# soberguo/HOIGen

Measured on AMD Instinct MI355X. Metric: union-crop embeddings/sec ViT-B/16 bs=256, higher is better.
Workload: dtype f16; 1 GPU; CLIP ViT-B/16 union-region encode (encode_image), 224x224 crops, batch 256 per GPU, synthetic N(0,1) crops + seeded synthetic weights (BASELINE.json configs[1]); last_block=all rows (option last_block_row0 = 0), batch_per_gpu=256, global_batch=256, parallelism=dp1

## Files before the change

hoigen_amd/csrc/hg_api.hip:

```cpp
#include <limits.h>

#include "hg_host.h"
#include "hg_preproc_geom.h"

namespace {

struct Option { const char *key, *env; int hg_ctx::*member; bool is_switch; int lo = 0, hi = 1; const char* want = nullptr; bool say_got = true; };
const Option OPTIONS[] = {
    {"chunk_rows", "HG_CHUNK_ROWS", &hg_ctx::max_chunk_rows, false, 256, INT_MAX, ">= 256", false},
    {"last_block_row0", "HG_LAST_BLOCK_ROW0", &hg_ctx::opt_row0, true},
    {"ln_fuse", "HG_LN_FUSE", &hg_ctx::opt_ln_fuse, true},
    {"adapter_fuse", "HG_ADAPTER_FUSE", &hg_ctx::opt_adapter_fuse, true},
    {"adapter_fold", "HG_ADAPTER_FOLD", &hg_ctx::opt_adapter_fold, true},
    {"stream_hilo", "HG_STREAM_HILO", &hg_ctx::opt_stream_hilo, true},
    {"adapter_long", "HG_ADAPTER_LONG", &hg_ctx::opt_adapter_long, true},
    {"qkv_attn", "HG_QKV_ATTN", &hg_ctx::opt_qkv_attn, false, 0, 2, "0, 1 or 2"},
    {"qkv_attn_text", "HG_QKV_ATTN_TEXT", &hg_ctx::opt_qkv_attn_text, false, 0, 2, "0, 1 or 2"},
    {"qkv_attn_min_seq", "HG_QKV_ATTN_MIN_SEQ", &hg_ctx::opt_qkv_attn_min_seq, false, 1, INT_MAX, ">= 1"},
    {"qkv_attn_gsz", "HG_QKV_ATTN_GSZ", &hg_ctx::opt_qkv_attn_gsz, false, 0, 6, "0 .. 6"},
    {"qkv_attn_c", "HG_QKV_ATTN_C", &hg_ctx::opt_qkv_attn_c, false, 0, 1, "0 or 1"},
    {"text_ln_fold", "HG_TEXT_LN_FOLD", &hg_ctx::opt_text_ln_fold, false, 0, 2, "0, 1 or 2"},
    {"vae_fused", "HG_VAE_FUSED", &hg_ctx::opt_vae_fused, false, 0, 2, "0, 1 or 2"},
    {"mlp_pair", "HG_MLP_PAIR", &hg_ctx::opt_mlp_pair, false, 0, 1, "0 or 1"},
    {"mlp_pair_chunk", "HG_MLP_PAIR_CHUNK", &hg_ctx::opt_mlp_pair_chunk, false, 1, 64, "1 .. 64"},
    {"mlp_pair_fc_slots", "HG_MLP_PAIR_FC_SLOTS", &hg_ctx::opt_mlp_pair_fc_slots, false, 1, 64, "1 .. 64"},
    {"mlp_pair256", "HG_MLP_PAIR256", &hg_ctx::opt_mlp_pair256, false, 0, 1, "0 or 1"},
    {"mlp_pair256_min_m", "HG_MLP_PAIR256_MIN_M", &hg_ctx::opt_mlp_pair256_min_m, false, 2048, INT_MAX, ">= 2048"},
    {"mlp_pair256_chunk", "HG_MLP_PAIR256_CHUNK", &hg_ctx::opt_mlp_pair256_chunk, false, 1, 64, "1 .. 64"},
    {"mlp_pair256_ratio", "HG_MLP_PAIR256_RATIO", &hg_ctx::opt_mlp_pair256_ratio, false, 1, 8, "1 .. 8"},
    {"mlp_pair256_launches", "HG_MLP_PAIR256_LAUNCHES", &hg_ctx::n_pair256_launches, false, 0, INT_MAX, ">= 0"},
    {"mlp_pair_fault", "HG_MLP_PAIR_FAULT", &hg_ctx::opt_mlp_pair_fault, false, 0, 1, "0 or 1"},
};
const Option* find_option(const char* key) {
    for (const Option& o : OPTIONS)
        if (!strcmp(o.key, key)) return &o;
    return nullptr;
}

}

extern "C" {

const char* hg_version(void) { return "hoigen_amd 0.1 (gfx950)"; }

// ... 245 lines not shown
```

hoigen_amd/csrc/hg_gemm_ring_body.h:

```cpp
#pragma once
#include <type_traits>

#include "hg_gemm_dev.h"

namespace hg {

#ifdef HG_STAMPS
#ifndef HG_STAMP_MASK
#define HG_STAMP_MASK 0xFF
#endif
#define SEG_B(k) do { if constexpr ((HG_STAMP_MASK >> (k)) & 1) t_beg = __builtin_amdgcn_s_memtime(); } while (0)
#define SEG_E(k) do { if constexpr ((HG_STAMP_MASK >> (k)) & 1) tacc[k] += __builtin_amdgcn_s_memtime() - t_beg; } while (0)
#else
#define SEG_B(k) do {} while (0)
#define SEG_E(k) do {} while (0)
#endif

template <int MF, int EPI, bool PH2, int HL = 0, class SCHED>
__device__ __forceinline__ void gemm_ring_body(const GemmArgs& p, const unsigned a_bytes, const int mode, const SCHED& sc) {
#if defined(__HIP_DEVICE_COMPILE__)
    constexpr int BM = 64 * MF, BK = 64;
    constexpr int AH = MF * 4096, BH = 16384;
    constexpr int STAGE = 2 * AH + 2 * BH;
    constexpr int GA = MF / 2, GB = 2;
    static_assert(GA <= 2, "DMA piece helpers cover two pieces per half-tile");
    constexpr int N1 = 2 * GA + 3 * GB, N2 = 3 * GA + 2 * GB;
    constexpr bool RLN = (EPI == EPI_RESID_LN_F32);
    constexpr bool RESID = (EPI == EPI_BIAS_RESID_F32 || EPI == EPI_SCALE_RESID_F32 || RLN);
    constexpr bool F16_STORES = (EPI == EPI_BIAS_F16 || EPI == EPI_BIAS_QGELU_F16 || EPI == EPI_BIAS_RELU_F16 ||
                                 EPI == EPI_LN_BIAS_F16 || EPI == EPI_LN_BIAS_QGELU_F16);
    constexpr bool IN_HL = (HL == 2 || HL == 3), OUT_HL = (HL == 2);
    static_assert(HL == 0 || (IN_HL && RLN && MF == 4 && !PH2), "hi / lo stream: EPI_RESID_LN_F32 on 256 rows, four phases, hl 2 or 3");
    constexpr int E_RAW = IN_HL ? (OUT_HL ? 40 : 88) : RLN ? 8 * MF + 4 * MF + 2 * MF : (F16_STORES ? 4 * MF : 8 * MF);
    constexpr int E = E_RAW > 52 ? 52 : E_RAW;
    constexpr bool XPRE = RESID && MF == 2;
    constexpr bool LNC = (EPI == EPI_LN_BIAS_F16 || EPI == EPI_LN_BIAS_QGELU_F16);
    constexpr bool ROLL = RESID && MF == 4;
    constexpr int ROLL_W = RLN ? 6 : 8;
    constexpr int R = XPRE ? E : (IN_HL ? 12 : ROLL ? ROLL_W + (RLN ? 1 : 0) : 0);
    constexpr bool PUB = SCHED::PUBLISH;
    static_assert(!PUB || (PH2 && (EPI == EPI_LN_BIAS_F16 || EPI == EPI_LN_BIAS_QGELU_F16)), "hand-off: two-phase loop, fp16 LayerNorm-fold epilogues");
    constexpr int BIAS_OFF = 2 * STAGE;
    const int MR_OFF = BIAS_OFF + 2 * p.N * 4;
    extern __shared__ __attribute__((aligned(16))) char smem[];
#ifdef HG_STAMPS
    unsigned long long tacc[8] = {0, 0, 0, 0, 0, 0, 0, 0}, t_beg = 0, t_all = 0;
#endif
    const int tid = sc.thread_id(), lane = tid & 63;
    const int wave = __builtin_amdgcn_readfirstlane(tid >> 6);
    const int wm = wave >> 2, wn = wave & 3;
    const int nk = p.K / BK;

    const int bid = blockIdx.x;
    const int n_items = sc.n_items();
    const int my_tiles = n_items;
    const int tiles_m_all = (p.M + BM - 1) / BM;
    auto item_get = [&](int e, int& tm, int& tn, int& kb, int& ke) {
        kb = 0;
        ke = nk;
        sc.tile(e, tm, tn);
    };
    {
        const int dunit = mode >> 8;
// ... 78 lines not shown
    half8 xa[MF][2], wb[2][2][2];
    auto read_A = [&](int h, int buf) {
#pragma unroll
        for (int f = 0; f < MF; ++f)
#pragma unroll
            for (int ks = 0; ks < 2; ++ks)
                xa[f][ks] = *reinterpret_cast<const half8*>(smem + buf + h * AH + a_row + f * 2048 + coff[ks]);
    };
    auto read_W = [&](auto H, int buf) {
        constexpr int h = decltype(H)::value;
#pragma unroll
        for (int g2 = 0; g2 < 2; ++g2)
#pragma unroll
            for (int ks = 0; ks < 2; ++ks)
                wb[h][g2][ks] = *reinterpret_cast<const half8*>(smem + buf + h * BH + w_row + g2 * 2048 + coff[ks]);
    };

    f32x4 acc[2][2][MF][2];
    auto zero_acc = [&]() {
#pragma unroll
        for (int a = 0; a < 2; ++a)
#pragma unroll
            for (int b = 0; b < 2; ++b)
#pragma unroll
                for (int f = 0; f < MF; ++f)
#pragma unroll
                    for (int g2 = 0; g2 < 2; ++g2) acc[a][b][f][g2] = f32x4{0.f, 0.f, 0.f, 0.f};
    };
    auto mma = [&](auto HA, auto HB) {
        constexpr int ha = decltype(HA)::value, hb = decltype(HB)::value;
// ... 111 lines not shown
            }
        };
        auto chunk_row = [&](int rg) {
            int m = m0 + (rg / MF) * (BM / 2) + wm * MF * 16 + (rg % MF) * 16 + (lane & 15);
            return m < p.M ? m : p.M - 1;
        };
        auto chunk_load = [&](int c) {
            const int rg = c >> 2, hb = (c >> 1) & 1, g2 = c & 1;
            const int n = n0 + hb * 128 + wn * 32 + g2 * 16 + 4 * (lane >> 4);
            return *reinterpret_cast<const f32x4*>(reinterpret_cast<const float*>(p.out) + (size_t)chunk_row(rg) * p.ldc + n);
        };
        auto ph2_ktile = [&](auto KIND_T) {
            constexpr int KINDX = decltype(KIND_T)::value;
            constexpr int KIND = KINDX >= 4 ? 0 : KINDX;
            const int buf = (g & 1) * STAGE;
            const bool post = post_ok;
            const bool more = KIND < 2 || r + 1 < n_items;
            const bool pub = PUB && r > 0 && wave == 0;
            (void)post; (void)more; (void)pub;
            constexpr int NP = 2 * GA + 2 * GB;
            read_A(0, buf);
            read_W(I0{}, buf);
            read_W(I1{}, buf);
            if constexpr (LNC && KIND == 2) {
                if (lane < BM / 16)
                    __builtin_amdgcn_raw_ptr_buffer_load_lds(rsM, (HG_LDS void*)(smem + MR_OFF + wave * BM), 16, lane * 16,
                                                             (m0 + wave * (BM / 8)) * 8, 0, 0);
            }
            if (KIND < 3 || more) issue_A(1, 0, GA);
            if constexpr (ROLL && KIND == 3) {
                {
#pragma unroll
                    for (int c = 0; c < ROLL_W; ++c) xw[c] = chunk_load(c);
                    if constexpr (RLN) muw[0] = p.mu[chunk_row(0)];
                }
            }
            if constexpr (XPRE && KIND == 3) {
                {
#pragma unroll
                    for (int ha = 0; ha < 2; ++ha)
#pragma unroll
                        for (int f = 0; f < MF; ++f) {
                            int m = m0 + ha * (BM / 2) + wm * MF * 16 + f * 16 + (lane & 15);
                            m = m < p.M ? m : p.M - 1;
#pragma unroll
                            for (int hb = 0; hb < 2; ++hb)
#pragma unroll
                                for (int g2 = 0; g2 < 2; ++g2) {
                                    const int n = n0 + hb * 128 + wn * 32 + g2 * 16 + 4 * (lane >> 4);
                                    xres[ha][hb][f][g2] = *reinterpret_cast<const f32x4*>(
                                        reinterpret_cast<const float*>(p.out) + (size_t)m * p.ldc + n);
                                }
                        }
                }
            }
            SEG_B(0);
            if constexpr (KINDX == 5) { if (pub) wait_vm<NP + 1>(); else wait_vm<NP>(); }
            else if constexpr (KIND == 0) wait_vm<NP>();
            else if constexpr (KIND == 1) { if (post) wait_vm<NP + E>(); else wait_vm<NP>(); }
            else if constexpr (KIND == 2) { if (more) wait_vm<NP>(); else wait_vm<0>(); }
            else { if (more) wait_vm<NP + R>(); else wait_vm<0>(); }
            SEG_E(0);
            sync_fetch();
            mma(I0{}, I0{});
            mma(I0{}, I1{});
            sync_mma();
            if constexpr (KINDX == 4) {
                if (pub) sc.publish(tm_prev, lane);
            }
            read_A(1, buf);
            if (KIND < 2 || more) { ld_advance(std::integral_constant<int, KIND == 2 ? 1 : 0>{}); issue_A(0, 0, GA); issue_W(0, 0, GB); issue_W(1, 0, GB); }
            SEG_B(0);
            if constexpr (KINDX == 4) { if (pub) wait_vm<NP + 1>(); else wait_vm<NP>(); }
            else if constexpr (KIND == 0) wait_vm<NP>();
            else if constexpr (KIND == 1) { if (post) wait_vm<NP + E>(); else wait_vm<NP>(); }
            else if constexpr (KIND == 2) { if (more) wait_vm<NP>(); else wait_vm<0>(); }
            else { if (more) wait_vm<NP + R>(); else wait_vm<0>(); }
            SEG_E(0);
            sync_fetch();
            mma(I1{}, I1{});
            mma(I1{}, I0{});
            sync_mma();
            ++g;
        };
        if constexpr (PH2) {
            using K0 = std::integral_constant<int, 0>;
            using K1 = std::integral_constant<int, 1>;
            using K2 = std::integral_constant<int, 2>;
            using K3 = std::integral_constant<int, 3>;
            ph2_ktile(K1{});
            if constexpr (PUB) {
                ph2_ktile(std::integral_constant<int, 4>{});
                ph2_ktile(std::integral_constant<int, 5>{});
            }
            for (int kt = PUB ? 3 : 1; kt < klen - 2; ++kt) {
                ph2_ktile(K0{});
            }
            ph2_ktile(K2{});
            ph2_ktile(K3{});
        } else {
        for (int kt = 0; kt < klen; ++kt, ++g) {
            const int buf = (g & 1) * STAGE;
            const bool more = g + 2 < S;
            const bool post = post_ok;
            const bool xl = (XPRE || ROLL) && kt == klen - 1;
            read_A(0, buf);
            read_W(I0{}, buf);
            if constexpr (LNC) {
                if (kt == klen - 2 && lane < BM / 16)
                    __builtin_amdgcn_raw_ptr_buffer_load_lds(rsM, (HG_LDS void*)(smem + MR_OFF + wave * BM), 16, lane * 16,
                                                             (m0 + wave * (BM / 8)) * 8, 0, 0);
            }
            if (g + 1 < S) issue_A(1, 0, GA);
            if constexpr (IN_HL) {
// ... 359 lines not shown
```

hoigen_amd/csrc/hg_host.h:

```cpp
#pragma once
#include <math.h>
#include <stdarg.h>
#include <stdio.h>
#include <stdlib.h>
#include <string.h>

#include <algorithm>
#include <string>
#include <vector>

#include "../../include/hoigen_amd.h"
#include "hg_kernels.h"

using namespace hg;

namespace hg_host {
struct Buf {
    void* p = nullptr;
    size_t bytes = 0;
};

struct BlockW {
    half_t *w_qkv, *w_out, *w_fc, *w_proj;
    float *b_qkv, *b_out, *b_fc, *b_proj, *ln1_w, *ln1_b, *ln2_w, *ln2_b;
// ... 120 lines not shown
    int opt_qkv_attn = 1;
    int opt_qkv_attn_min_seq = 32;
    int opt_qkv_attn_gsz = 0;
    int opt_text_ln_fold = 1;
    int opt_adapter_long = 0;
    int opt_qkv_attn_text = 0;
    int opt_qkv_attn_c = 1;
    int opt_vae_fused = 1;
    int opt_mlp_pair = 1;
    int opt_mlp_pair_chunk = 32;
    int opt_mlp_pair_fc_slots = 32;
    int opt_mlp_pair256 = 1;
    int opt_mlp_pair256_min_m = 25000;
    int opt_mlp_pair256_chunk = 6;
    int opt_mlp_pair256_ratio = 4;
    int n_pair256_launches = 0;
    int opt_mlp_pair_fault = 0;
    int n_cu = 256;
    int32_t* pair_err = nullptr;
    int32_t* range_flag = nullptr;
    int32_t* eot_flag = nullptr;
    int32_t* eot_flag_dev = nullptr;
    int prof_kind = HG_PROF_OFF;
    std::vector<hipEvent_t> prof_ev;
    std::vector<hg_prof_rec> prof_rec;
    size_t prof_n = 0;
};

namespace hg_host {
#define HG_WORKSPACE_BUFS(c)                                                                                                          \
// ... 106 lines not shown
```

hoigen_amd/csrc/hg_kernels.h:

```cpp
#pragma once
#include <hip/hip_runtime.h>
#include <stdint.h>

#include "hg_common.h"

namespace hg {

enum Epilogue : int {
    EPI_BIAS_F16 = 0,
    EPI_BIAS_QGELU_F16 = 1,
    EPI_BIAS_RELU_F16 = 2,
    EPI_BIAS_RESID_F32 = 3,
    EPI_BIAS_F32 = 4,
    EPI_PATCH_F32 = 5,
    EPI_BIAS_RELU_F32 = 6,
    EPI_SCALE_RESID_F32 = 7,
    EPI_LN_BIAS_F16 = 8,
    EPI_LN_BIAS_QGELU_F16 = 9,
    EPI_RESID_LN_F32 = 10,
    EPI_MU_BIAS_RELU_F32 = 11,
    EPI_SCALE_RESID_LN_F32 = 12
};

#ifndef HG_LO_SCALE
// ... 25 lines not shown
    const float* gamma = nullptr;
    half_t* out3 = nullptr;
    int ld3 = 0;
};
inline size_t gemm_lo_bytes(int M, int N) { return (size_t)((M + 127) / 128) * (N / 256) * 65536; }

hipError_t launch_gemm(int epi, const GemmArgs& a, hipStream_t s);
double gemm_flops(const GemmArgs& a);
bool gemm_ring_ok(const GemmArgs& a);
hipError_t launch_gemm_ring(int epi, const GemmArgs& a, hipStream_t s);
bool gemm_ring2_ok(const GemmArgs& a);
bool gemm_ln_ok(int epi, const GemmArgs& a);
hipError_t launch_gemm_ring2(int epi, const GemmArgs& a, hipStream_t s);
hipError_t launch_gemm_simple(int epi, const GemmArgs& a, hipStream_t s);
bool mlp_pair_ok(const GemmArgs& fc, const GemmArgs& proj, int n_cu);
size_t mlp_pair_ready_words(int M);
hipError_t launch_mlp_pair(const GemmArgs& fc, const GemmArgs& proj, unsigned* ready, int* err, int ch, int fc_slots, int n_cu, hipStream_t s,
                           int grid_short = 0);
bool mlp_pair256_ok(const GemmArgs& fc, const GemmArgs& proj, int n_cu, int min_m);
hipError_t launch_mlp_pair256(const GemmArgs& fc, const GemmArgs& proj, unsigned* ready, int* err, int ch, int ratio, int n_cu,
                              hipStream_t s, int grid_short = 0);
bool gemm_duo_ok(int epi, const GemmArgs& a);
hipError_t launch_gemm_duo(int epi, const GemmArgs& a, hipStream_t s);

static constexpr int ATTN_MAX_L_RESIDENT = 224;
static constexpr int ATTN_LONG_MAX_L = 640;
hipError_t launch_attention(const half_t* qkv, half_t* out, int n_seq, int L, int heads, bool causal,
                            hipStream_t s, int ldo = 0, bool pack = true);
hipError_t launch_attention_row0(const half_t* qkv, const half_t* q0, const int32_t* sel, half_t* out, int n_seq, int L,
                                 int heads, bool causal, hipStream_t s);
hipError_t launch_attention_long(const half_t* qkv, half_t* out, int n_seq, int L, int heads, bool causal, hipStream_t s, int ldo);
hipError_t launch_attention_long_row0(const half_t* qkv, const half_t* q0, const int32_t* sel, half_t* out, int n_seq, int L,
                                      int heads, bool causal, hipStream_t s);

struct QkvAttnArgs {
    const half_t* x16 = nullptr;
// ... 231 lines not shown
```

hoigen_amd/csrc/hg_mlp_pair.hip:

```cpp
#include "hg_gemm_ring_body.h"
#include "hg_gemm_ring2_body.h"
#include "hg_mlp_pair_dev.h"

namespace hg {

struct MlpFcSched {
    static constexpr bool PUBLISH = true, CONSUME = false;
    MlpFcList list;
    MlpFcDeal deal;
    int wave;
    unsigned* ready;
    __device__ __forceinline__ MlpFcSched(const MlpGeom& g, int M, int N, unsigned* ready_)
        : list(g.xcd, g.ch, N / 256, mlp_panels((M + 255) / 256, g.xcd)), deal(list.size(), g.cu, g.fcs) {
        wave = g.wave; ready = ready_;
    }
    __device__ __forceinline__ int n_items() const { return deal.total; }
    __device__ __forceinline__ int slack() const { return deal.slack(); }
    __device__ __forceinline__ void tile(int r, int& tm, int& tn_) const { list.tile(deal.pos(r), tm, tn_); }
    __device__ __forceinline__ int thread_id() const { return mlp_thread_id(wave); }
    __device__ __forceinline__ void publish(int tm, int lane) const {
        if (lane == 0) __hip_atomic_fetch_add(ready + tm, 1u, __ATOMIC_RELAXED, __HIP_MEMORY_SCOPE_AGENT);
    }
};

// ... 68 lines not shown
            barrier_raw();
            gemm_ring2_body<EPI_RESID_LN_F32, HL, GS>(a, a.N / 256, Q.a_bytes, 0, sp);
        }
#ifdef HG_STAMPS
        t_stamp[2] = __builtin_amdgcn_s_memtime();
        if (P.dbg && threadIdx.x == 0) {
            unsigned long long* d = P.dbg + (size_t)blockIdx.x * 8;
            d[0] = t_stamp[0]; d[1] = t_stamp[1]; d[2] = t_stamp[2]; d[3] = t_stamp[3]; d[4] = (unsigned long long)sp.deal.total;
            d[5] = (unsigned long long)(geo.xcd * 256 + geo.cu);
        }
#endif
    }
#endif
}

bool mlp_pair_ok(const GemmArgs& fc, const GemmArgs& proj, int n_cu) {
    if (n_cu != 32 * MLP_NX) return false;
    if (!gemm_ln_ok(EPI_LN_BIAS_QGELU_F16, fc) || !gemm_ln_ok(EPI_RESID_LN_F32, proj)) return false;
    if (fc.M != proj.M || proj.K != fc.N || proj.lda != fc.ldc || (const void*)proj.A != fc.out) return false;
    if (fc.K < 5 * 64 || proj.K < 8 * 64) return false;
    if ((size_t)((fc.M + 255) / 256) * 256 * fc.ldc * 2 >= (1ull << 32)) return false;
    if (fc.M < 8 * 256) return false;
    if (proj.gamma && proj.hl == 2 && (!proj.out3 || proj.ld3 < proj.N || (proj.ld3 % 8))) return false;
    return proj.hl == 0 || proj.hl == 2 || proj.hl == 3;
}

static hipError_t launch_pair_hl(const MlpPairArgs& a, int hl, bool gs, int grid, int lds, hipStream_t s) {
    if (gs) {
        switch (hl) {
            case 2: return mlp_launch_instance<mlp_pair_kernel<2, true>>(a, grid, lds, s);
            case 3: return mlp_launch_instance<mlp_pair_kernel<3, true>>(a, grid, lds, s);
            default: return hipErrorInvalidValue;
        }
    }
    switch (hl) {
        case 0: return mlp_launch_instance<mlp_pair_kernel<0, false>>(a, grid, lds, s);
        case 2: return mlp_launch_instance<mlp_pair_kernel<2, false>>(a, grid, lds, s);
// ... 33 lines not shown
```

hoigen_amd/csrc/hg_mlp_pair256.hip:

```cpp
#include <limits.h>

#include "hg_gemm_ring_body.h"
#include "hg_mlp_pair_dev.h"

namespace hg {

struct Pair256FcSched {
    static constexpr bool PUBLISH = true, CONSUME = false;
    int x, ch, tn, wave, npx, total, slack_t;
    Pair256Deal deal;
    unsigned* ready;
    __device__ __forceinline__ Pair256FcSched(const MlpGeom& g, int M, int N, int proj_tn, int ratio, unsigned* ready_)
        : deal(mlp_panels((M + 255) / 256, g.xcd) * (N / 256), mlp_panels((M + 255) / 256, g.xcd) * proj_tn, g.cpx, g.cu, ratio) {
        x = g.xcd; ch = g.ch; wave = g.wave; ready = ready_;
        tn = N / 256;
        npx = mlp_panels((M + 255) / 256, x);
        total = deal.n_fc();
        slack_t = deal.slack();
    }
    __device__ __forceinline__ int n_items() const { return total; }
    __device__ __forceinline__ int slack() const { return slack_t; }
    __device__ __forceinline__ void tile(int r, int& tm, int& tn_) const {
        const int L = deal.fc_pos(r);
        MlpFcList(x, ch, tn, npx).tile(L, tm, tn_);
    }
    __device__ __forceinline__ int thread_id() const { return mlp_thread_id(wave); }
    __device__ __forceinline__ void publish(int tm, int lane) const {
        if (lane == 0) __hip_atomic_fetch_add(ready + tm, 1u, __ATOMIC_RELAXED, __HIP_MEMORY_SCOPE_AGENT);
    }
};

struct Pair256ProjSched {
    static constexpr bool PUBLISH = false, CONSUME = true;
    int tm, tn, wave;
    __device__ __forceinline__ int n_items() const { return 1; }
    __device__ __forceinline__ int slack() const { return 0; }
    __device__ __forceinline__ void tile(int, int& tm_, int& tn_) const { tm_ = tm; tn_ = tn; }
    __device__ __forceinline__ int thread_id() const { return mlp_thread_id(wave); }
    __device__ __forceinline__ void publish(int, int) const {}
};

struct Pair256Args {
    MlpFcArgs fc;
    MlpProjArgs proj;
    unsigned* ready;
    int* err;
    int ch;
    int proj_tn;
    int ratio;
    int census_off;
    unsigned long long* dbg;
};

template <int HL>
__global__ __launch_bounds__(512, 2) void mlp_pair256_kernel(const Pair256Args P_in) {
#if defined(__HIP_DEVICE_COMPILE__)
    extern __shared__ __attribute__((aligned(16))) char smem[];
    const Pair256Args& P = P_in;
    MlpGeom geo;
    if (!mlp_take_slot(geo, smem, P.ready, P.census_off, P.ch, INT_MAX)) return;
#ifdef HG_STAMPS
    unsigned long long t_stamp[4] = {__builtin_amdgcn_s_memtime(), 0, 0, 0};
#endif
    {
        Pair256FcSched sf(geo, P.fc.M, P.fc.N, P.proj_tn, P.ratio, P.ready + MLP_CENSUS);
        if (sf.total > 0) {
            const GemmArgs a = mlp_fc_gemm_args(P.fc);
            gemm_ring_body<4, EPI_LN_BIAS_QGELU_F16, true>(a, P.fc.a_bytes, 3000 << 8, sf);
        }
#ifdef HG_STAMPS
        t_stamp[1] = __builtin_amdgcn_s_memtime();
        t_stamp[3] = (unsigned long long)sf.total;
#endif
    }
    {
        const int tnp = P.proj_tn, npx = mlp_panels((P.fc.M + 255) / 256, geo.xcd);
        const Pair256Deal deal(npx * (P.fc.N / 256), npx * tnp, geo.cpx, geo.cu, P.ratio);
        const int n_proj = deal.n_proj(), item0 = deal.proj_item(0);
        for (int j = 0; j < n_proj; ++j) {
            const MlpProjArgs Q = load_kernarg<MlpProjArgs>((unsigned)__builtin_offsetof(Pair256Args, proj));
            const GemmArgs a = mlp_proj_gemm_args<false>(Q);
            const int i = item0 + j * geo.cpx;
            Pair256ProjSched sp;
            sp.wave = geo.wave;
            pair256_proj_tile(i, geo.xcd, tnp, sp.tm, sp.tn);
            if (geo.wave == 0) mlp_wait_panel(P.ready + MLP_CENSUS + sp.tm, (unsigned)(P.fc.N / 256), P.err);
            __builtin_amdgcn_s_waitcnt(0xC07F);
            barrier_raw();
            gemm_ring_body<4, EPI_RESID_LN_F32, false, HL>(a, Q.a_bytes, 0, sp);
        }
#ifdef HG_STAMPS
        t_stamp[2] = __builtin_amdgcn_s_memtime();
        if (P.dbg && threadIdx.x == 0) {
            unsigned long long* d = P.dbg + (size_t)blockIdx.x * 8;
            d[0] = t_stamp[0]; d[1] = t_stamp[1]; d[2] = t_stamp[2]; d[3] = t_stamp[3]; d[4] = (unsigned long long)n_proj;
            d[5] = (unsigned long long)(geo.xcd * 256 + geo.cu);
        }
#endif
    }
#endif
}

bool mlp_pair256_ok(const GemmArgs& fc, const GemmArgs& proj, int n_cu, int min_m) {
    if (!mlp_pair_ok(fc, proj, n_cu) || proj.gamma) return false;
    if (fc.M < min_m) return false;
    if ((size_t)((proj.M + 255) / 256) * 256 * proj.lda * 2 >= (1ull << 31)) return false;
    return proj.hl == 0 || proj.hl == 2 || proj.hl == 3;
}

static hipError_t launch_pair256_hl(const Pair256Args& a, int hl, int grid, int lds, hipStream_t s) {
    switch (hl) {
        case 0: return mlp_launch_instance<mlp_pair256_kernel<0>>(a, grid, lds, s);
        case 2: return mlp_launch_instance<mlp_pair256_kernel<2>>(a, grid, lds, s);
        case 3: return mlp_launch_instance<mlp_pair256_kernel<3>>(a, grid, lds, s);
        default: return hipErrorInvalidValue;
    }
}

hipError_t launch_mlp_pair256(const GemmArgs& fc, const GemmArgs& proj_in, unsigned* ready, int* err, int ch, int ratio, int n_cu,
                              hipStream_t s, int grid_short) {
    GemmArgs proj = proj_in;
    if (!proj.ld2) proj.ld2 = proj.ldc;
    if (!mlp_pair256_ok(fc, proj, n_cu, 0) || !ready || !err || proj.ld2 % 8) return hipErrorInvalidValue;
    if (proj.hl && (!proj.lo || !proj.mu || !proj.muc)) return hipErrorInvalidValue;
    Pair256Args a{};
    mlp_pack_args(fc, proj, 256, a.fc, a.proj);
    a.ready = ready; a.err = err;
    a.ch = ch < 1 ? 1 : (ch > 64 ? 64 : ch);
    a.proj_tn = proj.N / 256;
    a.ratio = ratio < 1 ? 1 : (ratio > 8 ? 8 : ratio);
    const int lds = mlp_pair_lds(fc.N, 2 * (2 * 4 * 4096 + 2 * 16384) + proj.N * 4, a.census_off);
    if (!lds) return hipErrorInvalidValue;
    const int grid = mlp_pair_grid(n_cu, grid_short);
    auto launch = [&](unsigned long long* dbg) {
        a.dbg = dbg;
        return launch_pair256_hl(a, proj.hl, grid, lds, s);
    };
#ifdef HG_STAMPS
    if (getenv("HG_STAMPS")) return mlp_launch_stamped("pair256", grid, s, launch);
#endif
    return launch(nullptr);
}

}
```

hoigen_amd/csrc/hg_tower.hip:

```cpp
#include <mutex>

#include "hg_host.h"

namespace {

struct PairGate {
    std::mutex mu;
    bool have_first = false, multi = false, evt_set = false;
    hipStream_t first = nullptr;
    hipEvent_t evt = nullptr;
};
static PairGate g_pair_gate[16];
struct PairGateScope {
    PairGate* g;
    hipStream_t s;
    PairGateScope(int dev, hipStream_t s_) : g(&g_pair_gate[dev & 15]), s(s_) {
        g->mu.lock();
        if (!g->have_first) { g->first = s; g->have_first = true; }
        else if (!g->multi && s != g->first) {
            (void)hipDeviceSynchronize();
            if (hipEventCreateWithFlags(&g->evt, hipEventDisableTiming) != hipSuccess) g->evt = nullptr;
            g->multi = true;
        }
        if (g->multi && g->evt && g->evt_set) (void)hipStreamWaitEvent(s, g->evt, 0);
// ... 249 lines not shown
        b.hl_proj = b.emits ? hl_at(p.hilo, 2 * (int)i + 1, n_rln) : 0;
        b.x_hilo = p.hilo && (b.emits ? b.hl_proj : b.hl_out) != 3;
        b.x16 = b.fold ? p.att : p.h;
        b.ldx = b.fold ? D + 64 : D;
        b.a1 = !p.gs ? b.x16 : i == 0 ? p.hg : ln_copy(p, p.blocks[i - 1].hl_proj);
        b.a2 = p.hilo_c ? p.att : ln_copy(p, b.hl_out);
        b.lda2 = p.hilo_c ? D + 64 : D;
        const bool qa = !b.row0 && blocks[i].wp_qkv && (b.fold ? qa_cat && b.fold->wp_qcat : qa_on);
        const bool qat = qat_on && !b.row0 && (p.gs ? blocks[i].wpg_qkv : blocks[i].wp_qkv);
        b.in_proj = !p.fuse ? InProj::separate : b.fold ? (qa ? InProj::qkv_attn_cat : InProj::cat) :
                    qa ? InProj::qkv_attn : qat ? InProj::qkv_attn_text : InProj::folded;
    }
    for (size_t i = 0; p.pair_on && i + 1 < nb; ++i) {
        const GemmArgs fc = fc_args(p, blocks[i], p.blocks[i], D);
        const GemmArgs proj = proj_args(p, blocks[i], p.blocks[i], D, &p.blocks[i + 1], blocks[i + 1].ln1_w);
        p.blocks[i].pair = mlp_pair_ok(fc, proj, c->n_cu);
        p.blocks[i].pair256 = p.blocks[i].pair && c->opt_mlp_pair256 && !t.causal && mlp_pair256_ok(fc, proj, c->n_cu, c->opt_mlp_pair256_min_m);
    }
    p.pre16 = !t.pre_w ? (p.gs ? p.hg : p.h) : nb ? p.blocks[0].x16 : p.h;
    p.pre_ld = t.pre_w && nb ? p.blocks[0].ldx : D;
    return HG_OK;
}

int check_sticky_flags(hg_ctx* c) {
    if (c->pair_err && *(volatile int32_t*)c->pair_err) {
        *(volatile int32_t*)c->pair_err = 0;
        if (c->range_flag) *(volatile int32_t*)c->range_flag = 0;
        return fail(c, HG_ERR_HIP, "a hand-off wait inside the MLP pair kernel of a previous call timed out (a workgroup of its grid never "
                                   "became resident): that call's outputs are invalid; set option mlp_pair = 0 if this device cannot "
                                   "hold one workgroup per compute unit");
    }
    if (c->range_flag && *(volatile int32_t*)c->range_flag) {
// ... 60 lines not shown
}

int launch_mlp(hg_ctx* c, const TowerCall& t, const TowerPlan& p, const std::vector<BlockW>& blocks, size_t i) {
    const BlockW& w = blocks[i];
    const BlockPlan& b = p.blocks[i];
    const int D = t.D;
    hipStream_t s = t.s;
    if (!p.fuse) HG_HIP(launch_layernorm_f16(p.x, w.ln2_w, w.ln2_b, p.h, p.M, D, nullptr, 0, 1, s));
    const GemmArgs fc = fc_args(p, w, b, D);
    const GemmArgs proj = proj_args(p, w, b, D, b.emits ? &p.blocks[i + 1] : nullptr, b.emits ? blocks[i + 1].ln1_w : nullptr);
    if (b.pair) {
        PairGateScope gate(c->device, s);
        ProfScope ps(c, s, HG_PROF_MLP_PAIR, p.M, 4 * D, D);
        unsigned* ready = (unsigned*)c->pair_ready.p + i * (size_t)p.pair_panels;
        if (b.pair256) ++c->n_pair256_launches;
        if (b.pair256)
            HG_HIP(launch_mlp_pair256(fc, proj, ready, c->pair_err, c->opt_mlp_pair256_chunk, c->opt_mlp_pair256_ratio, c->n_cu, s, c->opt_mlp_pair_fault));
        else
            HG_HIP(launch_mlp_pair(fc, proj, ready, c->pair_err, c->opt_mlp_pair_chunk, c->opt_mlp_pair_fc_slots, c->n_cu, s, c->opt_mlp_pair_fault));
    } else {
        HG_HIP(gemm(c, p.fuse ? EPI_LN_BIAS_QGELU_F16 : EPI_BIAS_QGELU_F16, fc, s));
        if (w.w_proj_lo && b.adapter && !p.hilo) {
            GemmArgs lo = gemm_args(p.fc, 4 * D, w.w_proj_lo, c->vit.lo_scale + D, p.x, D, p.M, D, 4 * D);
            lo.pos = c->vit.lo_scale;
            HG_HIP(gemm(c, EPI_SCALE_RESID_F32, lo, s));
        }
        HG_HIP(gemm(c, b.emits ? EPI_RESID_LN_F32 : EPI_BIAS_RESID_F32, proj, s));
    }
    if (b.emits) HG_HIP(launch_finalize_stats(p.stats, p.mr, p.mu, p.M, p.sld, 64, s, p.muc, false, c->range_flag));
    return HG_OK;
}
// ... 367 lines not shown
```

Before: 26600 crops/s.

## Run pair256 projection tiles through the two-phase ring loop with pinned LDS reads

Adds a pair256p MLP pair kernel variant, selected by a new mlp_pair256_ph2 option that defaults to on. In it, the projection GEMM (residual plus LayerNorm epilogue) runs on the two-phase pipelined ring loop instead of the four-phase one, specialised for exactly one tile per call. Its LDS fragment reads use inline-asm ds_read_b128 into fixed VGPR tuples, and the tail waits are retuned. The aim is to overlap the projection's K-loop more tightly and cut register pressure and scheduling slack. It also relaxes the minimum-M gates and shares the pair256 kernel body through a new header. The hard-coded register allocation and hand-written wait counts risk miscompiles or hazards if the compiler's own allocation clashes with them.

```diff
diff --git a/hoigen_amd/csrc/hg_api.hip b/hoigen_amd/csrc/hg_api.hip
--- a/hoigen_amd/csrc/hg_api.hip
+++ b/hoigen_amd/csrc/hg_api.hip
@@ -25,9 +25,10 @@
     {"mlp_pair_chunk", "HG_MLP_PAIR_CHUNK", &hg_ctx::opt_mlp_pair_chunk, false, 1, 64, "1 .. 64"},
     {"mlp_pair_fc_slots", "HG_MLP_PAIR_FC_SLOTS", &hg_ctx::opt_mlp_pair_fc_slots, false, 1, 64, "1 .. 64"},
     {"mlp_pair256", "HG_MLP_PAIR256", &hg_ctx::opt_mlp_pair256, false, 0, 1, "0 or 1"},
-    {"mlp_pair256_min_m", "HG_MLP_PAIR256_MIN_M", &hg_ctx::opt_mlp_pair256_min_m, false, 2048, INT_MAX, ">= 2048"},
+    {"mlp_pair256_min_m", "HG_MLP_PAIR256_MIN_M", &hg_ctx::opt_mlp_pair256_min_m, false, 256, INT_MAX, ">= 256"},
     {"mlp_pair256_chunk", "HG_MLP_PAIR256_CHUNK", &hg_ctx::opt_mlp_pair256_chunk, false, 1, 64, "1 .. 64"},
     {"mlp_pair256_ratio", "HG_MLP_PAIR256_RATIO", &hg_ctx::opt_mlp_pair256_ratio, false, 1, 8, "1 .. 8"},
+    {"mlp_pair256_ph2", "HG_MLP_PAIR256_PH2", &hg_ctx::opt_mlp_pair256_ph2, false, 0, 1, "0 or 1"},
     {"mlp_pair256_launches", "HG_MLP_PAIR256_LAUNCHES", &hg_ctx::n_pair256_launches, false, 0, INT_MAX, ">= 0"},
     {"mlp_pair_fault", "HG_MLP_PAIR_FAULT", &hg_ctx::opt_mlp_pair_fault, false, 0, 1, "0 or 1"},
 };
diff --git a/hoigen_amd/csrc/hg_gemm_ring_body.h b/hoigen_amd/csrc/hg_gemm_ring_body.h
--- a/hoigen_amd/csrc/hg_gemm_ring_body.h
+++ b/hoigen_amd/csrc/hg_gemm_ring_body.h
@@ -15,6 +15,21 @@
 #define SEG_B(k) do {} while (0)
 #define SEG_E(k) do {} while (0)
 #endif
+
+template <int I, int OFF, class T>
+__device__ __forceinline__ void ds_read_fixed(T& x, int addr) {
+    static_assert(sizeof(T) == 16 && I >= 0 && I < 16 && OFF >= 0 && OFF < 65536, "a 4-register fragment, 16 tuples, a 16-bit offset");
+#define HG_DS_READ_FIXED(n, r) if constexpr (I == n) asm volatile("ds_read_b128 %0, %1 offset:%2" : "={" r "}"(x) : "v"(addr), "n"(OFF) : "memory")
+    HG_DS_READ_FIXED(0, "v[192:195]"); HG_DS_READ_FIXED(1, "v[196:199]"); HG_DS_READ_FIXED(2, "v[200:203]"); HG_DS_READ_FIXED(3, "v[204:207]");
+    HG_DS_READ_FIXED(4, "v[208:211]"); HG_DS_READ_FIXED(5, "v[212:215]"); HG_DS_READ_FIXED(6, "v[216:219]"); HG_DS_READ_FIXED(7, "v[220:223]");
+    HG_DS_READ_FIXED(8, "v[224:227]"); HG_DS_READ_FIXED(9, "v[228:231]"); HG_DS_READ_FIXED(10, "v[232:235]"); HG_DS_READ_FIXED(11, "v[236:239]");
+    HG_DS_READ_FIXED(12, "v[240:243]"); HG_DS_READ_FIXED(13, "v[244:247]"); HG_DS_READ_FIXED(14, "v[248:251]"); HG_DS_READ_FIXED(15, "v[252:255]");
+#undef HG_DS_READ_FIXED
+}
+template <class F, int... I>
+__device__ __forceinline__ void static_for_impl(F&& f, std::integer_sequence<int, I...>) { (f(std::integral_constant<int, I>{}), ...); }
+template <int N, class F>
+__device__ __forceinline__ void static_for(F&& f) { static_for_impl(f, std::make_integer_sequence<int, N>{}); }
 
 template <int MF, int EPI, bool PH2, int HL = 0, class SCHED>
 __device__ __forceinline__ void gemm_ring_body(const GemmArgs& p, const unsigned a_bytes, const int mode, const SCHED& sc) {
@@ -30,7 +45,9 @@
     constexpr bool F16_STORES = (EPI == EPI_BIAS_F16 || EPI == EPI_BIAS_QGELU_F16 || EPI == EPI_BIAS_RELU_F16 ||
                                  EPI == EPI_LN_BIAS_F16 || EPI == EPI_LN_BIAS_QGELU_F16);
     constexpr bool IN_HL = (HL == 2 || HL == 3), OUT_HL = (HL == 2);
-    static_assert(HL == 0 || (IN_HL && RLN && MF == 4 && !PH2), "hi / lo stream: EPI_RESID_LN_F32 on 256 rows, four phases, hl 2 or 3");
+    static_assert(HL == 0 || (IN_HL && RLN && MF == 4), "hi / lo stream: EPI_RESID_LN_F32 on 256 rows, hl 2 or 3");
+    constexpr bool ONE = PH2 && SCHED::CONSUME;
+    static_assert(!(PH2 && RLN) || (ONE && MF == 4), "two-phase loop under EPI_RESID_LN_F32: one tile per call, 256 rows");
     constexpr int E_RAW = IN_HL ? (OUT_HL ? 40 : 88) : RLN ? 8 * MF + 4 * MF + 2 * MF : (F16_STORES ? 4 * MF : 8 * MF);
     constexpr int E = E_RAW > 52 ? 52 : E_RAW;
     constexpr bool XPRE = RESID && MF == 2;
@@ -46,7 +63,8 @@
 #ifdef HG_STAMPS
     unsigned long long tacc[8] = {0, 0, 0, 0, 0, 0, 0, 0}, t_beg = 0, t_all = 0;
 #endif
-    const int tid = sc.thread_id(), lane = tid & 63;
+    const int tid = sc.thread_id();
+    int lane = tid & 63;
     const int wave = __builtin_amdgcn_readfirstlane(tid >> 6);
     const int wm = wave >> 2, wn = wave & 3;
     const int nk = p.K / BK;
@@ -155,6 +173,23 @@
 #pragma unroll
             for (int ks = 0; ks < 2; ++ks)
                 wb[h][g2][ks] = *reinterpret_cast<const half8*>(smem + buf + h * BH + w_row + g2 * 2048 + coff[ks]);
+    };
+
+    auto read_A_fixed = [&](auto H, int buf) {
+        constexpr int h = decltype(H)::value;
+        const int base = (int)(unsigned)(__SIZE_TYPE__)(HG_LDS char*)smem + buf + a_row;
+        static_for<2 * MF>([&](auto I) {
+            constexpr int f = decltype(I)::value >> 1, ks = decltype(I)::value & 1;
+            if constexpr (MF == 4) ds_read_fixed<f * 2 + ks, h * AH + f * 2048>(xa[f][ks], base + coff[ks]);
+        });
+    };
+    auto read_W_fixed = [&](auto H, int buf) {
+        constexpr int h = decltype(H)::value;
+        const int base = (int)(unsigned)(__SIZE_TYPE__)(HG_LDS char*)smem + buf + w_row;
+        static_for<4>([&](auto I) {
+            constexpr int g2 = decltype(I)::value >> 1, ks = decltype(I)::value & 1;
+            ds_read_fixed<8 + h * 4 + g2 * 2 + ks, h * BH + g2 * 2048>(wb[h][g2][ks], base + coff[ks]);
+        });
     };
 
     f32x4 acc[2][2][MF][2];
@@ -296,21 +331,28 @@
             constexpr int KINDX = decltype(KIND_T)::value;
             constexpr int KIND = KINDX >= 4 ? 0 : KINDX;
             const int buf = (g & 1) * STAGE;
-            const bool post = post_ok;
-            const bool more = KIND < 2 || r + 1 < n_items;
+            const bool post = !ONE && post_ok;
+            const bool more = KIND < 2 || (!ONE && r + 1 < n_items);
             const bool pub = PUB && r > 0 && wave == 0;
             (void)post; (void)more; (void)pub;
             constexpr int NP = 2 * GA + 2 * GB;
-            read_A(0, buf);
-            read_W(I0{}, buf);
-            read_W(I1{}, buf);
+            if constexpr (ONE) {
+                read_A_fixed(I0{}, buf);
+                read_W_fixed(I0{}, buf);
+                read_W_fixed(I1{}, buf);
+            } else {
+                read_A(0, buf);
+                read_W(I0{}, buf);
+                read_W(I1{}, buf);
+            }
             if constexpr (LNC && KIND == 2) {
                 if (lane < BM / 16)
                     __builtin_amdgcn_raw_ptr_buffer_load_lds(rsM, (HG_LDS void*)(smem + MR_OFF + wave * BM), 16, lane * 16,
                                                              (m0 + wave * (BM / 8)) * 8, 0, 0);
             }
             if (KIND < 3 || more) issue_A(1, 0, GA);
-            if constexpr (ROLL && KIND == 3) {
+            if constexpr (IN_HL && KIND == 3) unit_load(0);
+            if constexpr (ROLL && !IN_HL && KIND == 3) {
                 {
 #pragma unroll
                     for (int c = 0; c < ROLL_W; ++c) xw[c] = chunk_load(c);
@@ -340,8 +382,8 @@
             if constexpr (KINDX == 5) { if (pub) wait_vm<NP + 1>(); else wait_vm<NP>(); }
             else if constexpr (KIND == 0) wait_vm<NP>();
             else if constexpr (KIND == 1) { if (post) wait_vm<NP + E>(); else wait_vm<NP>(); }
-            else if constexpr (KIND == 2) { if (more) wait_vm<NP>(); else wait_vm<0>(); }
-            else { if (more) wait_vm<NP + R>(); else wait_vm<0>(); }
+            else if constexpr (KIND == 2) { if (more) wait_vm<NP>(); else wait_vm<ONE ? NP : 0>(); }
+            else { if (more) wait_vm<NP + R>(); else wait_vm<ONE ? R : 0>(); }
             SEG_E(0);
             sync_fetch();
             mma(I0{}, I0{});
@@ -350,14 +392,15 @@
             if constexpr (KINDX == 4) {
                 if (pub) sc.publish(tm_prev, lane);
             }
-            read_A(1, buf);
+            if constexpr (ONE) read_A_fixed(I1{}, buf);
+            else read_A(1, buf);
             if (KIND < 2 || more) { ld_advance(std::integral_constant<int, KIND == 2 ? 1 : 0>{}); issue_A(0, 0, GA); issue_W(0, 0, GB); issue_W(1, 0, GB); }
             SEG_B(0);
             if constexpr (KINDX == 4) { if (pub) wait_vm<NP + 1>(); else wait_vm<NP>(); }
             else if constexpr (KIND == 0) wait_vm<NP>();
             else if constexpr (KIND == 1) { if (post) wait_vm<NP + E>(); else wait_vm<NP>(); }
-            else if constexpr (KIND == 2) { if (more) wait_vm<NP>(); else wait_vm<0>(); }
-            else { if (more) wait_vm<NP + R>(); else wait_vm<0>(); }
+            else if constexpr (KIND == 2) { if (more) wait_vm<NP>(); else wait_vm<ONE ? GA : 0>(); }
+            else { if (more) wait_vm<NP + R>(); else if constexpr (!ONE) wait_vm<0>(); }
             SEG_E(0);
             sync_fetch();
             mma(I1{}, I1{});
@@ -378,8 +421,10 @@
             for (int kt = PUB ? 3 : 1; kt < klen - 2; ++kt) {
                 ph2_ktile(K0{});
             }
+            if constexpr (ONE) lane = sc.thread_id() & 63;
             ph2_ktile(K2{});
             ph2_ktile(K3{});
+            if constexpr (ONE) asm volatile("" : "+v"(lane));
         } else {
         for (int kt = 0; kt < klen; ++kt, ++g) {
             const int buf = (g & 1) * STAGE;
diff --git a/hoigen_amd/csrc/hg_host.h b/hoigen_amd/csrc/hg_host.h
--- a/hoigen_amd/csrc/hg_host.h
+++ b/hoigen_amd/csrc/hg_host.h
@@ -158,6 +158,7 @@
     int opt_mlp_pair256_min_m = 25000;
     int opt_mlp_pair256_chunk = 6;
     int opt_mlp_pair256_ratio = 4;
+    int opt_mlp_pair256_ph2 = 1;
     int n_pair256_launches = 0;
     int opt_mlp_pair_fault = 0;
     int n_cu = 256;
diff --git a/hoigen_amd/csrc/hg_kernels.h b/hoigen_amd/csrc/hg_kernels.h
--- a/hoigen_amd/csrc/hg_kernels.h
+++ b/hoigen_amd/csrc/hg_kernels.h
@@ -63,12 +63,15 @@
 hipError_t launch_gemm_ring2(int epi, const GemmArgs& a, hipStream_t s);
 hipError_t launch_gemm_simple(int epi, const GemmArgs& a, hipStream_t s);
 bool mlp_pair_ok(const GemmArgs& fc, const GemmArgs& proj, int n_cu);
+bool mlp_pair_shapes_ok(const GemmArgs& fc, const GemmArgs& proj, int n_cu);
 size_t mlp_pair_ready_words(int M);
 hipError_t launch_mlp_pair(const GemmArgs& fc, const GemmArgs& proj, unsigned* ready, int* err, int ch, int fc_slots, int n_cu, hipStream_t s,
                            int grid_short = 0);
 bool mlp_pair256_ok(const GemmArgs& fc, const GemmArgs& proj, int n_cu, int min_m);
 hipError_t launch_mlp_pair256(const GemmArgs& fc, const GemmArgs& proj, unsigned* ready, int* err, int ch, int ratio, int n_cu,
                               hipStream_t s, int grid_short = 0);
+hipError_t launch_mlp_pair256p(const GemmArgs& fc, const GemmArgs& proj, unsigned* ready, int* err, int ch, int ratio, int n_cu,
+                               hipStream_t s, int grid_short = 0);
 bool gemm_duo_ok(int epi, const GemmArgs& a);
 hipError_t launch_gemm_duo(int epi, const GemmArgs& a, hipStream_t s);
 
diff --git a/hoigen_amd/csrc/hg_mlp_pair.hip b/hoigen_amd/csrc/hg_mlp_pair.hip
--- a/hoigen_amd/csrc/hg_mlp_pair.hip
+++ b/hoigen_amd/csrc/hg_mlp_pair.hip
@@ -106,13 +106,13 @@
 #endif
 }
 
-bool mlp_pair_ok(const GemmArgs& fc, const GemmArgs& proj, int n_cu) {
+bool mlp_pair_ok(const GemmArgs& fc, const GemmArgs& proj, int n_cu) { return fc.M >= 8 * 256 && mlp_pair_shapes_ok(fc, proj, n_cu); }
+bool mlp_pair_shapes_ok(const GemmArgs& fc, const GemmArgs& proj, int n_cu) {
     if (n_cu != 32 * MLP_NX) return false;
     if (!gemm_ln_ok(EPI_LN_BIAS_QGELU_F16, fc) || !gemm_ln_ok(EPI_RESID_LN_F32, proj)) return false;
     if (fc.M != proj.M || proj.K != fc.N || proj.lda != fc.ldc || (const void*)proj.A != fc.out) return false;
     if (fc.K < 5 * 64 || proj.K < 8 * 64) return false;
     if ((size_t)((fc.M + 255) / 256) * 256 * fc.ldc * 2 >= (1ull << 32)) return false;
-    if (fc.M < 8 * 256) return false;
     if (proj.gamma && proj.hl == 2 && (!proj.out3 || proj.ld3 < proj.N || (proj.ld3 % 8))) return false;
     return proj.hl == 0 || proj.hl == 2 || proj.hl == 3;
 }
diff --git a/hoigen_amd/csrc/hg_mlp_pair256.hip b/hoigen_amd/csrc/hg_mlp_pair256.hip
--- a/hoigen_amd/csrc/hg_mlp_pair256.hip
+++ b/hoigen_amd/csrc/hg_mlp_pair256.hip
@@ -1,108 +1,14 @@
-#include <limits.h>
-
-#include "hg_gemm_ring_body.h"
-#include "hg_mlp_pair_dev.h"
+#include "hg_mlp_pair256_dev.h"
 
 namespace hg {
 
-struct Pair256FcSched {
-    static constexpr bool PUBLISH = true, CONSUME = false;
-    int x, ch, tn, wave, npx, total, slack_t;
-    Pair256Deal deal;
-    unsigned* ready;
-    __device__ __forceinline__ Pair256FcSched(const MlpGeom& g, int M, int N, int proj_tn, int ratio, unsigned* ready_)
-        : deal(mlp_panels((M + 255) / 256, g.xcd) * (N / 256), mlp_panels((M + 255) / 256, g.xcd) * proj_tn, g.cpx, g.cu, ratio) {
-        x = g.xcd; ch = g.ch; wave = g.wave; ready = ready_;
-        tn = N / 256;
-        npx = mlp_panels((M + 255) / 256, x);
-        total = deal.n_fc();
-        slack_t = deal.slack();
-    }
-    __device__ __forceinline__ int n_items() const { return total; }
-    __device__ __forceinline__ int slack() const { return slack_t; }
-    __device__ __forceinline__ void tile(int r, int& tm, int& tn_) const {
-        const int L = deal.fc_pos(r);
-        MlpFcList(x, ch, tn, npx).tile(L, tm, tn_);
-    }
-    __device__ __forceinline__ int thread_id() const { return mlp_thread_id(wave); }
-    __device__ __forceinline__ void publish(int tm, int lane) const {
-        if (lane == 0) __hip_atomic_fetch_add(ready + tm, 1u, __ATOMIC_RELAXED, __HIP_MEMORY_SCOPE_AGENT);
-    }
-};
-
-struct Pair256ProjSched {
-    static constexpr bool PUBLISH = false, CONSUME = true;
-    int tm, tn, wave;
-    __device__ __forceinline__ int n_items() const { return 1; }
-    __device__ __forceinline__ int slack() const { return 0; }
-    __device__ __forceinline__ void tile(int, int& tm_, int& tn_) const { tm_ = tm; tn_ = tn; }
-    __device__ __forceinline__ int thread_id() const { return mlp_thread_id(wave); }
-    __device__ __forceinline__ void publish(int, int) const {}
-};
-
-struct Pair256Args {
-    MlpFcArgs fc;
-    MlpProjArgs proj;
-    unsigned* ready;
-    int* err;
-    int ch;
-    int proj_tn;
-    int ratio;
-    int census_off;
-    unsigned long long* dbg;
-};
-
 template <int HL>
 __global__ __launch_bounds__(512, 2) void mlp_pair256_kernel(const Pair256Args P_in) {
-#if defined(__HIP_DEVICE_COMPILE__)
-    extern __shared__ __attribute__((aligned(16))) char smem[];
-    const Pair256Args& P = P_in;
-    MlpGeom geo;
-    if (!mlp_take_slot(geo, smem, P.ready, P.census_off, P.ch, INT_MAX)) return;
-#ifdef HG_STAMPS
-    unsigned long long t_stamp[4] = {__builtin_amdgcn_s_memtime(), 0, 0, 0};
-#endif
-    {
-        Pair256FcSched sf(geo, P.fc.M, P.fc.N, P.proj_tn, P.ratio, P.ready + MLP_CENSUS);
-        if (sf.total > 0) {
-            const GemmArgs a = mlp_fc_gemm_args(P.fc);
-            gemm_ring_body<4, EPI_LN_BIAS_QGELU_F16, true>(a, P.fc.a_bytes, 3000 << 8, sf);
-        }
-#ifdef HG_STAMPS
-        t_stamp[1] = __builtin_amdgcn_s_memtime();
-        t_stamp[3] = (unsigned long long)sf.total;
-#endif
-    }
-    {
-        const int tnp = P.proj_tn, npx = mlp_panels((P.fc.M + 255) / 256, geo.xcd);
-        const Pair256Deal deal(npx * (P.fc.N / 256), npx * tnp, geo.cpx, geo.cu, P.ratio);
-        const int n_proj = deal.n_proj(), item0 = deal.proj_item(0);
-        for (int j = 0; j < n_proj; ++j) {
-            const MlpProjArgs Q = load_kernarg<MlpProjArgs>((unsigned)__builtin_offsetof(Pair256Args, proj));
-            const GemmArgs a = mlp_proj_gemm_args<false>(Q);
-            const int i = item0 + j * geo.cpx;
-            Pair256ProjSched sp;
-            sp.wave = geo.wave;
-            pair256_proj_tile(i, geo.xcd, tnp, sp.tm, sp.tn);
-            if (geo.wave == 0) mlp_wait_panel(P.ready + MLP_CENSUS + sp.tm, (unsigned)(P.fc.N / 256), P.err);
-            __builtin_amdgcn_s_waitcnt(0xC07F);
-            barrier_raw();
-            gemm_ring_body<4, EPI_RESID_LN_F32, false, HL>(a, Q.a_bytes, 0, sp);
-        }
-#ifdef HG_STAMPS
-        t_stamp[2] = __builtin_amdgcn_s_memtime();
-        if (P.dbg && threadIdx.x == 0) {
-            unsigned long long* d = P.dbg + (size_t)blockIdx.x * 8;
-            d[0] = t_stamp[0]; d[1] = t_stamp[1]; d[2] = t_stamp[2]; d[3] = t_stamp[3]; d[4] = (unsigned long long)n_proj;
-            d[5] = (unsigned long long)(geo.xcd * 256 + geo.cu);
-        }
-#endif
-    }
-#endif
+    mlp_pair256_run<HL, false>(P_in);
 }
 
 bool mlp_pair256_ok(const GemmArgs& fc, const GemmArgs& proj, int n_cu, int min_m) {
-    if (!mlp_pair_ok(fc, proj, n_cu) || proj.gamma) return false;
+    if (!mlp_pair_shapes_ok(fc, proj, n_cu) || proj.gamma) return false;
     if (fc.M < min_m) return false;
     if ((size_t)((proj.M + 255) / 256) * 256 * proj.lda * 2 >= (1ull << 31)) return false;
     return proj.hl == 0 || proj.hl == 2 || proj.hl == 3;
@@ -117,29 +23,9 @@
     }
 }
 
-hipError_t launch_mlp_pair256(const GemmArgs& fc, const GemmArgs& proj_in, unsigned* ready, int* err, int ch, int ratio, int n_cu,
+hipError_t launch_mlp_pair256(const GemmArgs& fc, const GemmArgs& proj, unsigned* ready, int* err, int ch, int ratio, int n_cu,
                               hipStream_t s, int grid_short) {
-    GemmArgs proj = proj_in;
-    if (!proj.ld2) proj.ld2 = proj.ldc;
-    if (!mlp_pair256_ok(fc, proj, n_cu, 0) || !ready || !err || proj.ld2 % 8) return hipErrorInvalidValue;
-    if (proj.hl && (!proj.lo || !proj.mu || !proj.muc)) return hipErrorInvalidValue;
-    Pair256Args a{};
-    mlp_pack_args(fc, proj, 256, a.fc, a.proj);
-    a.ready = ready; a.err = err;
-    a.ch = ch < 1 ? 1 : (ch > 64 ? 64 : ch);
-    a.proj_tn = proj.N / 256;
-    a.ratio = ratio < 1 ? 1 : (ratio > 8 ? 8 : ratio);
-    const int lds = mlp_pair_lds(fc.N, 2 * (2 * 4 * 4096 + 2 * 16384) + proj.N * 4, a.census_off);
-    if (!lds) return hipErrorInvalidValue;
-    const int grid = mlp_pair_grid(n_cu, grid_short);
-    auto launch = [&](unsigned long long* dbg) {
-        a.dbg = dbg;
-        return launch_pair256_hl(a, proj.hl, grid, lds, s);
-    };
-#ifdef HG_STAMPS
-    if (getenv("HG_STAMPS")) return mlp_launch_stamped("pair256", grid, s, launch);
-#endif
-    return launch(nullptr);
+    return mlp_pair256_launch("pair256", fc, proj, ready, err, ch, ratio, n_cu, s, grid_short, launch_pair256_hl);
 }
 
 }
diff --git a/hoigen_amd/csrc/hg_mlp_pair256_dev.h b/hoigen_amd/csrc/hg_mlp_pair256_dev.h
--- /dev/null
+++ b/hoigen_amd/csrc/hg_mlp_pair256_dev.h
@@ -0,0 +1,144 @@
+#pragma once
+#include <limits.h>
+
+#include "hg_gemm_ring_body.h"
+#include "hg_mlp_pair_dev.h"
+
+namespace hg {
+
+struct Pair256FcSched {
+    static constexpr bool PUBLISH = true, CONSUME = false;
+    int x, ch, tn, wave, npx, total, slack_t;
+    Pair256Deal deal;
+    unsigned* ready;
+    __device__ __forceinline__ Pair256FcSched(const MlpGeom& g, int M, int N, int proj_tn, int ratio, unsigned* ready_)
+        : deal(mlp_panels((M + 255) / 256, g.xcd) * (N / 256), mlp_panels((M + 255) / 256, g.xcd) * proj_tn, g.cpx, g.cu, ratio) {
+        x = g.xcd; ch = g.ch; wave = g.wave; ready = ready_;
+        tn = N / 256;
+        npx = mlp_panels((M + 255) / 256, x);
+        total = deal.n_fc();
+        slack_t = deal.slack();
+    }
+    __device__ __forceinline__ int n_items() const { return total; }
+    __device__ __forceinline__ int slack() const { return slack_t; }
+    __device__ __forceinline__ void tile(int r, int& tm, int& tn_) const {
+        const int L = deal.fc_pos(r);
+        MlpFcList(x, ch, tn, npx).tile(L, tm, tn_);
+    }
+    __device__ __forceinline__ int thread_id() const { return mlp_thread_id(wave); }
+    __device__ __forceinline__ void publish(int tm, int lane) const {
+        if (lane == 0) __hip_atomic_fetch_add(ready + tm, 1u, __ATOMIC_RELAXED, __HIP_MEMORY_SCOPE_AGENT);
+    }
+};
+
+template <bool FRESH_TID>
+struct Pair256ProjSchedT {
+    static constexpr bool PUBLISH = false, CONSUME = true;
+    int tm, tn, wave;
+    __device__ __forceinline__ int n_items() const { return 1; }
+    __device__ __forceinline__ int slack() const { return 0; }
+    __device__ __forceinline__ void tile(int, int& tm_, int& tn_) const { tm_ = tm; tn_ = tn; }
+    __device__ __forceinline__ int thread_id() const {
+        if constexpr (FRESH_TID) {
+            unsigned z = 0;
+            asm volatile("" : "+v"(z));
+            int t = wave * 64 + (int)__builtin_amdgcn_mbcnt_hi(~0u, __builtin_amdgcn_mbcnt_lo(~0u, z));
+            asm volatile("" : "+v"(t));
+            return t;
+        } else {
+            return mlp_thread_id(wave);
+        }
+    }
+    __device__ __forceinline__ void publish(int, int) const {}
+};
+using Pair256ProjSched = Pair256ProjSchedT<false>;
+
+struct Pair256Args {
+    MlpFcArgs fc;
+    MlpProjArgs proj;
+    unsigned* ready;
+    int* err;
+    int ch;
+    int proj_tn;
+    int ratio;
+    int census_off;
+    unsigned long long* dbg;
+};
+
+template <int HL, bool PROJ_PH2>
+__device__ __forceinline__ void mlp_pair256_run(const Pair256Args& P) {
+#if defined(__HIP_DEVICE_COMPILE__)
+    extern __shared__ __attribute__((aligned(16))) char smem[];
+    MlpGeom geo;
+    if (!mlp_take_slot(geo, smem, P.ready, P.census_off, P.ch, INT_MAX)) return;
+#ifdef HG_STAMPS
+    unsigned long long t_stamp[4] = {__builtin_amdgcn_s_memtime(), 0, 0, 0};
+#endif
+    {
+        Pair256FcSched sf(geo, P.fc.M, P.fc.N, P.proj_tn, P.ratio, P.ready + MLP_CENSUS);
+        if (sf.total > 0) {
+            const GemmArgs a = mlp_fc_gemm_args(P.fc);
+            gemm_ring_body<4, EPI_LN_BIAS_QGELU_F16, true>(a, P.fc.a_bytes, 3000 << 8, sf);
+        }
+#ifdef HG_STAMPS
+        t_stamp[1] = __builtin_amdgcn_s_memtime();
+        t_stamp[3] = (unsigned long long)sf.total;
+#endif
+    }
+    {
+        const int tnp = P.proj_tn, npx = mlp_panels((P.fc.M + 255) / 256, geo.xcd);
+        const Pair256Deal deal(npx * (P.fc.N / 256), npx * tnp, geo.cpx, geo.cu, P.ratio);
+        const int n_proj = deal.n_proj(), item0 = deal.proj_item(0);
+        for (int j = 0; j < n_proj; ++j) {
+            const MlpProjArgs Q = load_kernarg<MlpProjArgs>((unsigned)__builtin_offsetof(Pair256Args, proj));
+            const GemmArgs a = mlp_proj_gemm_args<false>(Q);
+            const int i = item0 + j * geo.cpx;
+            Pair256ProjSchedT<PROJ_PH2> sp;
+            sp.wave = geo.wave;
+            pair256_proj_tile(i, geo.xcd, tnp, sp.tm, sp.tn);
+            if (geo.wave == 0) mlp_wait_panel(P.ready + MLP_CENSUS + sp.tm, (unsigned)(P.fc.N / 256), P.err);
+            __builtin_amdgcn_s_waitcnt(0xC07F);
+            barrier_raw();
+            gemm_ring_body<4, EPI_RESID_LN_F32, PROJ_PH2, HL>(a, Q.a_bytes, 0, sp);
+        }
+#ifdef HG_STAMPS
+        t_stamp[2] = __builtin_amdgcn_s_memtime();
+        if (P.dbg && threadIdx.x == 0) {
+            unsigned long long* d = P.dbg + (size_t)blockIdx.x * 8;
+            d[0] = t_stamp[0]; d[1] = t_stamp[1]; d[2] = t_stamp[2]; d[3] = t_stamp[3]; d[4] = (unsigned long long)n_proj;
+            d[5] = (unsigned long long)(geo.xcd * 256 + geo.cu);
+        }
+#endif
+    }
+#endif
+}
+
+bool mlp_pair256_ok(const GemmArgs& fc, const GemmArgs& proj, int n_cu, int min_m);
+template <class LAUNCH_HL>
+hipError_t mlp_pair256_launch(const char* tag, const GemmArgs& fc, const GemmArgs& proj_in, unsigned* ready, int* err, int ch, int ratio,
+                              int n_cu, hipStream_t s, int grid_short, LAUNCH_HL launch_hl) {
+    GemmArgs proj = proj_in;
+    if (!proj.ld2) proj.ld2 = proj.ldc;
+    if (!mlp_pair256_ok(fc, proj, n_cu, 0) || !ready || !err || proj.ld2 % 8) return hipErrorInvalidValue;
+    if (proj.hl && (!proj.lo || !proj.mu || !proj.muc)) return hipErrorInvalidValue;
+    Pair256Args a{};
+    mlp_pack_args(fc, proj, 256, a.fc, a.proj);
+    a.ready = ready; a.err = err;
+    a.ch = ch < 1 ? 1 : (ch > 64 ? 64 : ch);
+    a.proj_tn = proj.N / 256;
+    a.ratio = ratio < 1 ? 1 : (ratio > 8 ? 8 : ratio);
+    const int lds = mlp_pair_lds(fc.N, 2 * (2 * 4 * 4096 + 2 * 16384) + proj.N * 4, a.census_off);
+    if (!lds) return hipErrorInvalidValue;
+    const int grid = mlp_pair_grid(n_cu, grid_short);
+    auto launch = [&](unsigned long long* dbg) {
+        a.dbg = dbg;
+        return launch_hl(a, proj.hl, grid, lds, s);
+    };
+#ifdef HG_STAMPS
+    if (getenv("HG_STAMPS")) return mlp_launch_stamped(tag, grid, s, launch);
+#endif
+    (void)tag;
+    return launch(nullptr);
+}
+
+}
diff --git a/hoigen_amd/csrc/hg_mlp_pair256p.hip b/hoigen_amd/csrc/hg_mlp_pair256p.hip
--- /dev/null
+++ b/hoigen_amd/csrc/hg_mlp_pair256p.hip
@@ -0,0 +1,24 @@
+#include "hg_mlp_pair256_dev.h"
+
+namespace hg {
+
+template <int HL>
+__global__ __launch_bounds__(512, 2) void mlp_pair256p_kernel(const Pair256Args P_in) {
+    mlp_pair256_run<HL, true>(P_in);
+}
+
+static hipError_t launch_pair256p_hl(const Pair256Args& a, int hl, int grid, int lds, hipStream_t s) {
+    switch (hl) {
+        case 0: return mlp_launch_instance<mlp_pair256p_kernel<0>>(a, grid, lds, s);
+        case 2: return mlp_launch_instance<mlp_pair256p_kernel<2>>(a, grid, lds, s);
+        case 3: return mlp_launch_instance<mlp_pair256p_kernel<3>>(a, grid, lds, s);
+        default: return hipErrorInvalidValue;
+    }
+}
+
+hipError_t launch_mlp_pair256p(const GemmArgs& fc, const GemmArgs& proj, unsigned* ready, int* err, int ch, int ratio, int n_cu,
+                               hipStream_t s, int grid_short) {
+    return mlp_pair256_launch("pair256p", fc, proj, ready, err, ch, ratio, n_cu, s, grid_short, launch_pair256p_hl);
+}
+
+}
diff --git a/hoigen_amd/csrc/hg_tower.hip b/hoigen_amd/csrc/hg_tower.hip
--- a/hoigen_amd/csrc/hg_tower.hip
+++ b/hoigen_amd/csrc/hg_tower.hip
@@ -287,8 +287,8 @@
     for (size_t i = 0; p.pair_on && i + 1 < nb; ++i) {
         const GemmArgs fc = fc_args(p, blocks[i], p.blocks[i], D);
         const GemmArgs proj = proj_args(p, blocks[i], p.blocks[i], D, &p.blocks[i + 1], blocks[i + 1].ln1_w);
-        p.blocks[i].pair = mlp_pair_ok(fc, proj, c->n_cu);
-        p.blocks[i].pair256 = p.blocks[i].pair && c->opt_mlp_pair256 && !t.causal && mlp_pair256_ok(fc, proj, c->n_cu, c->opt_mlp_pair256_min_m);
+        p.blocks[i].pair256 = c->opt_mlp_pair256 && !t.causal && mlp_pair256_ok(fc, proj, c->n_cu, c->opt_mlp_pair256_min_m);
+        p.blocks[i].pair = p.blocks[i].pair256 || mlp_pair_ok(fc, proj, c->n_cu);
     }
     p.pre16 = !t.pre_w ? (p.gs ? p.hg : p.h) : nb ? p.blocks[0].x16 : p.h;
     p.pre_ld = t.pre_w && nb ? p.blocks[0].ldx : D;
@@ -379,7 +379,9 @@
         ProfScope ps(c, s, HG_PROF_MLP_PAIR, p.M, 4 * D, D);
         unsigned* ready = (unsigned*)c->pair_ready.p + i * (size_t)p.pair_panels;
         if (b.pair256) ++c->n_pair256_launches;
-        if (b.pair256)
+        if (b.pair256 && c->opt_mlp_pair256_ph2)
+            HG_HIP(launch_mlp_pair256p(fc, proj, ready, c->pair_err, c->opt_mlp_pair256_chunk, c->opt_mlp_pair256_ratio, c->n_cu, s, c->opt_mlp_pair_fault));
+        else if (b.pair256)
             HG_HIP(launch_mlp_pair256(fc, proj, ready, c->pair_err, c->opt_mlp_pair256_chunk, c->opt_mlp_pair256_ratio, c->n_cu, s, c->opt_mlp_pair_fault));
         else
             HG_HIP(launch_mlp_pair(fc, proj, ready, c->pair_err, c->opt_mlp_pair_chunk, c->opt_mlp_pair_fc_slots, c->n_cu, s, c->opt_mlp_pair_fault));
```

Measured after the change: 26950 crops/s, median of 6. 1.01x the previous value.
